# KCL-BMEIS/VS_Seg

Measured on AMD Instinct MI355X. Metric: train_patches_per_sec_fwd_bwd_384x128x128, higher is better.
Workload: dtype bf16; 1 GPU; BASELINE config 2: 2.5D attention-UNet fwd + Dice_spvPA(attention+hardness) + bwd + Adam on random 384x128x128 patches, batch 4 per GPU, dropout 0.1, random-init weights; global_batch=4, patch=384x128x128, parallelism=dp1

## Files before the change

vs_seg_amd/csrc/bn_bwd.h:

```cpp
#pragma once
#include "common.h"

struct BnBwdC8 {
  float sc[8], sh[8], mu[8], k1i[8], kc[8], kd[8];
};

__device__ __forceinline__ void bn_bwd_consts(BnBwdC8& c, const float* __restrict__ mean, const float* __restrict__ invstd, const float* __restrict__ gamma, const float* __restrict__ scale,
                                              const float* __restrict__ shift, const float* __restrict__ mean_dz, const float* __restrict__ mean_dzx, int ch0, float inv_keep) {
#pragma unroll
  for (int j = 0; j < 8; ++j) {
    const float is = invstd[ch0 + j], k1 = gamma[ch0 + j] * is;
    c.sc[j] = scale[ch0 + j];
    c.sh[j] = shift[ch0 + j];
    c.mu[j] = mean[ch0 + j];
    c.k1i[j] = k1 * inv_keep;
    c.kc[j] = -(k1 * mean_dzx[ch0 + j]) * is;
    c.kd[j] = -(k1 * mean_dz[ch0 + j]);
  }
}

__device__ __forceinline__ void bn_fwd_act8(const f8& y, unsigned keep, float alpha, float inv_keep, const float (&sc)[8], const float (&sh)[8], f8& o) {
#pragma unroll
  for (int j = 0; j < 8; ++j) {
    float z = y.v[j] * sc[j] + sh[j];
    z = ((keep >> j) & 1u) ? z * inv_keep : 0.f;
    o.v[j] = z > 0.f ? z : alpha * z;
  }
}

__device__ __forceinline__ void bn_bwd_dy8(const f8& y, const f8& g, unsigned keep, float alpha, const BnBwdC8& c, f8& o) {
#pragma unroll
  for (int j = 0; j < 8; ++j) {
    const float z = y.v[j] * c.sc[j] + c.sh[j];
    const float dd = z > 0.f ? g.v[j] : alpha * g.v[j];
    const float t = ((keep >> j) & 1u) ? dd : 0.f;
    o.v[j] = __builtin_fmaf(c.k1i[j], t, __builtin_fmaf(c.kc[j], y.v[j] - c.mu[j], c.kd[j]));
  }
}

__device__ __forceinline__ f8 bf16x8_to_f8(const uint4 u) {
  return f8{{__uint_as_float(u.x << 16), __uint_as_float(u.x & 0xffff0000u), __uint_as_float(u.y << 16), __uint_as_float(u.y & 0xffff0000u),
             __uint_as_float(u.z << 16), __uint_as_float(u.z & 0xffff0000u), __uint_as_float(u.w << 16), __uint_as_float(u.w & 0xffff0000u)}};
}
__device__ __forceinline__ uint4 f8_to_bf16x8(const f8& a) {
  uint4 u;
  u.x = f2bf2(a.v[0], a.v[1]);
  u.y = f2bf2(a.v[2], a.v[3]);
  u.z = f2bf2(a.v[4], a.v[5]);
  u.w = f2bf2(a.v[6], a.v[7]);
  return u;
}
```

vs_seg_amd/csrc/elementwise.hip:

```cpp
#define VSSEG_NT_STORES
#define VSSEG_NT_LOADS
#include "common.h"
#include "bn_bwd.h"
#include <algorithm>
#include <type_traits>

#define DISPATCH_T(dtype, ...)                         \
  do {                                                 \
    if ((dtype) == VSSEG_F32) { typedef float T; __VA_ARGS__; } \
    else { typedef bf16_t T; __VA_ARGS__; }            \
  } while (0)

static inline int split_of(const vsseg_tensor& t) { return t.ptr2 ? t.csplit : 0x7fffffff; }
static inline bool two_part_ok(const vsseg_tensor& t) {
  return !t.ptr2 || (t.csplit > 0 && t.csplit < t.c && t.csplit % 16 == 0 && t.pitch >= t.csplit && t.pitch >= t.c - t.csplit);
}
#define VSSEG_ONE_PART(name, ...)                                                                     \
  do {                                                                                                \
    const vsseg_tensor* ts_[] = {__VA_ARGS__};                                                        \
    for (const vsseg_tensor* t_ : ts_) VSSEG_CHECK(!t_->ptr2, name ": two-part tensors are not supported here"); \
  } while (0)

static inline int block_for_cgs(int cgs) {
  int a = cgs, b = 64;
// ... 221 lines not shown
#pragma unroll
      for (int j = 0; j < 8; ++j) r.v[j] = x1 * w1[j] + b1[j];
    }
    bn_fwd_act8(x, keep, alpha, inv_keep, sc, sh, x);
    if constexpr (RES != 0) {
#pragma unroll
      for (int j = 0; j < 8; ++j) x.v[j] += r.v[j];
    }
    st8(out + v * op + c, x);
  }
}
static inline int bn_fwd_grid(int64_t items, int cgs) {
  int g = grid_for(items, 256, 16384);
  g = (g + cgs - 1) / cgs * cgs;
  return g;
}
extern "C" int vsseg_bn_act_fwd(vsseg_tensor y, const float* scale, const float* shift, const float* alpha, float p_drop, uint64_t seed, uint32_t salt,
                                vsseg_tensor res, int32_t has_res, vsseg_tensor out, uint8_t* keep_out, void* stream) {
  VSSEG_ONE_PART("vsseg_bn_act_fwd", &y, &res, &out);
  VSSEG_CHECK(y.ptr && out.ptr && scale && shift && alpha && y.c % 8 == 0 && y.pitch % 8 == 0 && out.pitch % 8 == 0 && out.c == y.c && out.dtype == y.dtype, "vsseg_bn_act_fwd: bad arguments");
  VSSEG_CHECK(!has_res || (res.ptr && res.dtype == y.dtype && res.c == y.c && res.pitch % 8 == 0), "vsseg_bn_act_fwd: bad residual");
  VSSEG_CHECK(p_drop >= 0.f && p_drop < 1.f, "vsseg_bn_act_fwd: dropout p out of range");
  int64_t nv = tensor_voxels(y);
  int cgs = y.c / 8;
  dim3 g(bn_fwd_grid(nv * cgs, cgs)), b(256);
  DISPATCH_T(y.dtype, if (has_res) hipLaunchKernelGGL((bn_act_fwd_kernel<T, 1>), g, b, 0, as_stream(stream), (const T*)y.ptr, y.pitch, scale, shift, alpha, p_drop, seed, salt, (const T*)res.ptr, res.pitch, (T*)out.ptr, out.pitch, cgs, nv, (const float*)nullptr, (const float*)nullptr, keep_out);
             else hipLaunchKernelGGL((bn_act_fwd_kernel<T, 0>), g, b, 0, as_stream(stream), (const T*)y.ptr, y.pitch, scale, shift, alpha, p_drop, seed, salt, (const T*)nullptr, 0, (T*)out.ptr, out.pitch, cgs, nv, (const float*)nullptr, (const float*)nullptr, keep_out));
  VSSEG_LAUNCH_CHECK("vsseg_bn_act_fwd");
  return VSSEG_OK;
}
extern "C" int vsseg_bn_act_fwd_res1(vsseg_tensor y, const float* scale, const float* shift, const float* alpha, float p_drop, uint64_t seed, uint32_t salt,
                                     const void* x1, const float* res_w, const float* res_b, vsseg_tensor out, uint8_t* keep_out, void* stream) {
  VSSEG_ONE_PART("vsseg_bn_act_fwd_res1", &y, &out);
  VSSEG_CHECK(y.ptr && out.ptr && scale && shift && alpha && x1 && res_w && res_b && y.c % 8 == 0 && y.pitch % 8 == 0 && out.pitch % 8 == 0 && out.c == y.c && out.dtype == y.dtype, "vsseg_bn_act_fwd_res1: bad arguments");
  VSSEG_CHECK(p_drop >= 0.f && p_drop < 1.f, "vsseg_bn_act_fwd_res1: dropout p out of range");
  int64_t nv = tensor_voxels(y);
  int cgs = y.c / 8;
  dim3 g(bn_fwd_grid(nv * cgs, cgs)), b(256);
  DISPATCH_T(y.dtype, hipLaunchKernelGGL((bn_act_fwd_kernel<T, 2>), g, b, 0, as_stream(stream), (const T*)y.ptr, y.pitch, scale, shift, alpha, p_drop, seed, salt, (const T*)x1, 0, (T*)out.ptr, out.pitch, cgs, nv, res_w, res_b, keep_out));
  VSSEG_LAUNCH_CHECK("vsseg_bn_act_fwd_res1");
  return VSSEG_OK;
}

__global__ void dropout_mask_kernel(float* mask, int64_t n8, float p, uint64_t seed, uint32_t salt) {
  if (p > 0.f) dropout_resolve_seed(seed, salt);
  for (int64_t i = blockIdx.x * (int64_t)blockDim.x + threadIdx.x; i < n8; i += (int64_t)gridDim.x * blockDim.x) {
    unsigned keep = p > 0.f ? dropout_keep8(seed, salt, (uint64_t)i, p) : 0xffu;
    for (int j = 0; j < 8; ++j) mask[i * 8 + j] = (float)((keep >> j) & 1u);
  }
}
extern "C" int vsseg_dropout_mask(float* mask, int64_t nvox, int32_t c, float p_drop, uint64_t seed, uint32_t salt, void* stream) {
  VSSEG_CHECK(mask && c % 8 == 0, "vsseg_dropout_mask: bad arguments");
  int64_t n8 = nvox * (c / 8);
  hipLaunchKernelGGL(dropout_mask_kernel, dim3(grid_for(n8, 256)), dim3(256), 0, as_stream(stream), mask, n8, p_drop, seed, salt);
  VSSEG_LAUNCH_CHECK("vsseg_dropout_mask");
  return VSSEG_OK;
}

struct BnBwdArgs {
  const float *mean, *invstd, *gamma, *beta, *scale, *shift, *alpha;
  float p_drop;
  uint64_t seed;
  uint32_t salt;
};
__device__ __forceinline__ float bn_bwd_elem8(const f8& y, const f8& da, int c, int64_t i, const BnBwdArgs& a, float alpha, f8& dz, f8& xh) {
  const float inv_keep = 1.f / (1.f - a.p_drop);
  unsigned keep = a.p_drop > 0.f ? dropout_keep8(a.seed, a.salt, (uint64_t)i, a.p_drop) : 0xffu;
  float dal = 0.f;
#pragma unroll
  for (int j = 0; j < 8; ++j) {
    float xhat = (y.v[j] - a.mean[c + j]) * a.invstd[c + j];
    float z = y.v[j] * a.scale[c + j] + a.shift[c + j];
    bool k = (keep >> j) & 1u;
    float d = k ? z * inv_keep : 0.f;
    float g = da.v[j];
    float dd = d > 0.f ? g : alpha * g;
    if (d < 0.f) dal += g * d;
    dz.v[j] = k ? dd * inv_keep : 0.f;
    xh.v[j] = xhat;
  }
  return dal;
}

template <typename T> struct Raw8;
template <> struct Raw8<bf16_t> {
  uint4 u;
  static __device__ __forceinline__ Raw8 ld(const bf16_t* p) {
    Raw8 r;
#ifdef VSSEG_NT_LOADS
    typedef unsigned u32x4 __attribute__((ext_vector_type(4)));
    const u32x4 t = __builtin_nontemporal_load(reinterpret_cast<const u32x4*>(p));
    r.u = make_uint4(t[0], t[1], t[2], t[3]);
#else
    r.u = *reinterpret_cast<const uint4*>(p);
#endif
    return r;
  }
  __device__ __forceinline__ f8 cvt() const {
    return f8{{__uint_as_float(u.x << 16), __uint_as_float(u.x & 0xffff0000u), __uint_as_float(u.y << 16), __uint_as_float(u.y & 0xffff0000u),
               __uint_as_float(u.z << 16), __uint_as_float(u.z & 0xffff0000u), __uint_as_float(u.w << 16), __uint_as_float(u.w & 0xffff0000u)}};
  }
};
template <> struct Raw8<float> {
  f8 v;
  static __device__ __forceinline__ Raw8 ld(const float* p) { Raw8 r; r.v = ld8(p); return r; }
  __device__ __forceinline__ f8 cvt() const { return v; }
};

template <typename T, int U>
__global__ __launch_bounds__(1024) void bn_act_bwd_reduce_kernel(const T* __restrict__ y, int yp, const T* __restrict__ dout, int dp, BnBwdArgs a, int cgs, int64_t nvox, double* __restrict__ sums, int stride, double* __restrict__ alpha_acc,
                                                               const uint8_t* __restrict__ keep_in, unsigned* fxflag) {
  extern __shared__ float red[];
  const int C = cgs * 8, RW = 3 * C + 1, nw = (blockDim.x + 63) >> 6;
  for (int i = threadIdx.x; i < nw * RW; i += blockDim.x) red[i] = 0.f;
  __syncthreads();
  const float alpha = *a.alpha;
  if (a.p_drop > 0.f && keep_in == nullptr) dropout_resolve_seed(a.seed, a.salt);
  const int64_t gt = blockIdx.x * (int64_t)blockDim.x + threadIdx.x, nthreads = (int64_t)gridDim.x * blockDim.x;
  const int cg = (int)(gt % cgs);
  const int c = cg * 8;
  float sc[8], sh[8], mu[8];
#pragma unroll
  for (int j = 0; j < 8; ++j) { sc[j] = a.scale[c + j]; sh[j] = a.shift[c + j]; mu[j] = a.mean[c + j]; }
  const bool drop = a.p_drop > 0.f;
  const float inv_keep = 1.f / (1.f - a.p_drop);
  float s1[8] = {0, 0, 0, 0, 0, 0, 0, 0}, s2[8] = {0, 0, 0, 0, 0, 0, 0, 0}, s3[8] = {0, 0, 0, 0, 0, 0, 0, 0}, dal = 0.f;
  const int64_t vstep = nthreads / cgs;
  auto one = [&](const f8& yy, const f8& da, unsigned keep) {
#pragma unroll
    for (int j = 0; j < 8; ++j) {
      const float z = yy.v[j] * sc[j] + sh[j];
      const bool k = (keep >> j) & 1u;
      const float d = k ? z * inv_keep : 0.f;
      const float g = da.v[j];
      const float dd = d > 0.f ? g : alpha * g;
      if (d < 0.f) dal += g * d;
      const float dz = k ? dd * inv_keep : 0.f;
      s1[j] += dz; s2[j] += dz * (yy.v[j] - mu[j]); s3[j] += g;
    }
  };
  auto sweep = [&](auto src_c) {
    constexpr int SRC = decltype(src_c)::value;
    auto mask_of = [&](int64_t vv) -> unsigned {
      if constexpr (SRC == 0) return 0xffu;
      else if constexpr (SRC == 1) return (unsigned)keep_in[vv * cgs + cg];
      else return dropout_keep8(a.seed, a.salt, (uint64_t)(vv * cgs + cg), a.p_drop);
    };
    int64_t v = gt / cgs;
    for (; v + (U - 1) * vstep < nvox; v += U * vstep) {
      Raw8<T> yv[U], dv[U];
      unsigned kp[U];
#pragma unroll
      for (int u = 0; u < U; ++u) { yv[u] = Raw8<T>::ld(y + (v + u * vstep) * yp + c); dv[u] = Raw8<T>::ld(dout + (v + u * vstep) * dp + c); kp[u] = mask_of(v + u * vstep); }
#pragma unroll
      for (int u = 0; u < U; ++u) one(yv[u].cvt(), dv[u].cvt(), kp[u]);
    }
    for (; v < nvox; v += vstep) one(ld8(y + v * yp + c), ld8(dout + v * dp + c), mask_of(v));
  };
  if (!drop) sweep(std::integral_constant<int, 0>{});
  else if (keep_in != nullptr) sweep(std::integral_constant<int, 1>{});
  else sweep(std::integral_constant<int, 2>{});
  float* rw = red + (threadIdx.x >> 6) * RW;
#pragma unroll
  for (int j = 0; j < 8; ++j) { atomicAdd(&rw[c + j], s1[j]); atomicAdd(&rw[C + c + j], s2[j]); atomicAdd(&rw[2 * C + c + j], s3[j]); }
  dal = wave_sum(dal);
  if ((threadIdx.x & 63) == 0) rw[3 * C] = dal;
  __syncthreads();
  auto wsum = [&](int i) { float v = 0.f; for (int w = 0; w < nw; ++w) v += red[w * RW + i]; return v; };
  const int shard = blockIdx.x % VSSEG_STAT_SHARDS;
  for (int i = threadIdx.x; i < 3 * C; i += blockDim.x) {
    const int which = i / C, ch = i % C;
    double val = (double)wsum(i);
    if (which == 1) val *= (double)a.invstd[ch];
    vsseg_fx_add(&sums[(int64_t)shard * 3 * stride + which * stride + ch], val, VSSEG_FX_GRAD, fxflag);
  }
  if (threadIdx.x == 0) vsseg_fx_add(&alpha_acc[shard], (double)wsum(3 * C), VSSEG_FX_GRAD, fxflag);
}
extern "C" int vsseg_bn_act_bwd_reduce(vsseg_tensor y, vsseg_tensor dout, const float* mean, const float* invstd, const float* gamma, const float* beta, const float* scale, const float* shift, const float* alpha,
                                       float p_drop, uint64_t seed, uint32_t salt, double* sums, int32_t stride, double* alpha_acc, const uint8_t* keep_in, void* stream) {
  VSSEG_ONE_PART("vsseg_bn_act_bwd_reduce", &y, &dout);
  VSSEG_CHECK(y.ptr && dout.ptr && y.dtype == dout.dtype && y.c == dout.c && y.c % 8 == 0 && y.pitch % 8 == 0 && dout.pitch % 8 == 0 && sums && alpha_acc && stride >= y.c, "vsseg_bn_act_bwd_reduce: bad arguments");
  int cgs = y.c / 8, blk = block_for_cgs(cgs);
  VSSEG_CHECK(blk > 0, "vsseg_bn_act_bwd_reduce: unsupported channel count %d", y.c);
  int64_t nv = tensor_voxels(y);
  BnBwdArgs a{mean, invstd, gamma, beta, scale, shift, alpha, p_drop, seed, salt};
  size_t lds = (size_t)((blk + 63) / 64) * (3 * y.c + 1) * sizeof(float);
  const int64_t items = nv * cgs;
  const int budget = 65536;
  const int cap = (int)std::min<int64_t>(256 * 8, std::max<int64_t>(192, std::min<int64_t>(items / ((int64_t)blk * 16), y.c <= 16 ? 256 * 3 : budget / (3 * y.c))));
  int grid = grid_for((nv * cgs + 1) / 2, blk, cap);
  VSSEG_FX_FLAG(fxflag, "vsseg_bn_act_bwd_reduce");
  DISPATCH_T(y.dtype, hipLaunchKernelGGL((bn_act_bwd_reduce_kernel<T, 2>), dim3(grid), dim3(blk), lds, as_stream(stream), (const T*)y.ptr, y.pitch, (const T*)dout.ptr, dout.pitch, a, cgs, nv, sums, stride, alpha_acc, keep_in, fxflag));
  VSSEG_LAUNCH_CHECK("vsseg_bn_act_bwd_reduce");
  return VSSEG_OK;
}

__global__ void bn_act_bwd_finalize_kernel(const double* __restrict__ sums, int stride, const double* __restrict__ alpha_acc, int c, double count, float* dgamma, float* dbeta, float* dalpha, float* mean_dz, float* mean_dzx, float* dres_bias, const unsigned* fxflag) {
  __shared__ double part[4];
  const int ch = blockIdx.x, sh = threadIdx.x;
  const double* base = sums + (int64_t)sh * 3 * stride + ch;
  const double s = block256_sum_d(vsseg_fx_get(&base[0], VSSEG_FX_GRAD), part) + vsseg_fx_poison(fxflag);
  const double q = block256_sum_d(vsseg_fx_get(&base[stride], VSSEG_FX_GRAD), part) + vsseg_fx_poison(fxflag);
  const double r = block256_sum_d(vsseg_fx_get(&base[2 * stride], VSSEG_FX_GRAD), part) + vsseg_fx_poison(fxflag);
  double a = 0.0;
  if (ch == 0) a = block256_sum_d(vsseg_fx_get(&alpha_acc[sh], VSSEG_FX_GRAD), part);
  if (threadIdx.x != 0) return;
  if (ch == 0) *dalpha += (float)(a + vsseg_fx_poison(fxflag));
  if (dres_bias) dres_bias[ch] += (float)r;
  dbeta[ch] += (float)s;
  dgamma[ch] += (float)q;
  mean_dz[ch] = (float)(s / count);
  mean_dzx[ch] = (float)(q / count);
}
extern "C" int vsseg_bn_act_bwd_finalize(const double* sums, int32_t stride, const double* alpha_acc, int32_t c, double count, float* dgamma, float* dbeta, float* dalpha,
                                         float* mean_dz, float* mean_dzx, float* dres_bias, void* stream) {
  VSSEG_CHECK(sums && alpha_acc && dgamma && dbeta && dalpha && mean_dz && mean_dzx && c > 0, "vsseg_bn_act_bwd_finalize: bad arguments");
  VSSEG_FX_FLAG(fxflag, "vsseg_bn_act_bwd_finalize");
  hipLaunchKernelGGL(bn_act_bwd_finalize_kernel, dim3(c), dim3(256), 0, as_stream(stream), sums, stride, alpha_acc, c, count, dgamma, dbeta, dalpha, mean_dz, mean_dzx, dres_bias, fxflag);
  VSSEG_LAUNCH_CHECK("vsseg_bn_act_bwd_finalize");
  return VSSEG_OK;
}

template <typename T>
__global__ void bn_act_bwd_apply_kernel(const T* __restrict__ y, int yp, const T* __restrict__ dout, int dp, BnBwdArgs a, const float* __restrict__ mean_dz, const float* __restrict__ mean_dzx,
                                        T* __restrict__ dy, int dyp, int cgs, int64_t nvox, const uint8_t* __restrict__ keep_in) {
  const int64_t gt = blockIdx.x * (int64_t)blockDim.x + threadIdx.x, nthreads = (int64_t)gridDim.x * blockDim.x;
  const int cg = (int)(gt % cgs), c = cg * 8;
  const int64_t vstep = nthreads / cgs;
  const float alpha = *a.alpha, inv_keep = 1.f / (1.f - a.p_drop);
  BnBwdC8 k;
  bn_bwd_consts(k, a.mean, a.invstd, a.gamma, a.scale, a.shift, mean_dz, mean_dzx, c, inv_keep);
  const bool drop = a.p_drop > 0.f;
  if (drop && keep_in == nullptr) dropout_resolve_seed(a.seed, a.salt);
  auto one = [&](const f8& yy, const f8& da, unsigned keep, int64_t v) {
    f8 o;
    bn_bwd_dy8(yy, da, keep, alpha, k, o);
    st8(dy + v * dyp + c, o);
  };
  auto sweep = [&](auto src_c) {
    constexpr int SRC = decltype(src_c)::value;
    auto mask_of = [&](int64_t vv) -> unsigned {
      if constexpr (SRC == 0) return 0xffu;
      else if constexpr (SRC == 1) return (unsigned)keep_in[vv * cgs + cg];
      else return dropout_keep8(a.seed, a.salt, (uint64_t)(vv * cgs + cg), a.p_drop);
    };
    int64_t v = gt / cgs;
    for (; v + vstep < nvox; v += 2 * vstep) {
      const f8 y0 = ld8(y + v * yp + c), d0 = ld8(dout + v * dp + c);
      const f8 y1 = ld8(y + (v + vstep) * yp + c), d1 = ld8(dout + (v + vstep) * dp + c);
      const unsigned m0 = mask_of(v), m1 = mask_of(v + vstep);
      one(y0, d0, m0, v);
      one(y1, d1, m1, v + vstep);
    }
    if (v < nvox) one(ld8(y + v * yp + c), ld8(dout + v * dp + c), mask_of(v), v);
  };
  if (!drop) sweep(std::integral_constant<int, 0>{});
  else if (keep_in != nullptr) sweep(std::integral_constant<int, 1>{});
  else sweep(std::integral_constant<int, 2>{});
}

extern "C" int vsseg_bn_act_bwd_apply(vsseg_tensor y, vsseg_tensor dout, const float* mean, const float* invstd, const float* gamma, const float* beta, const float* scale, const float* shift, const float* alpha,
                                      float p_drop, uint64_t seed, uint32_t salt, const float* mean_dz, const float* mean_dzx, vsseg_tensor dy, const uint8_t* keep_in, void* stream) {
  VSSEG_ONE_PART("vsseg_bn_act_bwd_apply", &y, &dout, &dy);
  VSSEG_CHECK(y.ptr && dout.ptr && dy.ptr && y.dtype == dout.dtype && y.dtype == dy.dtype && y.c == dout.c && y.c == dy.c && y.c % 8 == 0 && y.pitch % 8 == 0 && dout.pitch % 8 == 0 && dy.pitch % 8 == 0,
              "vsseg_bn_act_bwd_apply: bad arguments");
  int cgs = y.c / 8, blk = block_for_cgs(cgs);
  VSSEG_CHECK(blk > 0, "vsseg_bn_act_bwd_apply: unsupported channel count %d", y.c);
  int64_t nv = tensor_voxels(y);
  BnBwdArgs a{mean, invstd, gamma, beta, scale, shift, alpha, p_drop, seed, salt};
  DISPATCH_T(y.dtype, hipLaunchKernelGGL(bn_act_bwd_apply_kernel<T>, dim3(grid_for((nv * cgs + 1) / 2, blk, 256 * 8)), dim3(blk), 0, as_stream(stream), (const T*)y.ptr, y.pitch, (const T*)dout.ptr, dout.pitch, a, mean_dz, mean_dzx, (T*)dy.ptr, dy.pitch, cgs, nv, keep_in));
  VSSEG_LAUNCH_CHECK("vsseg_bn_act_bwd_apply");
  return VSSEG_OK;
}

template <typename T>
__global__ void att_apply_fwd_kernel(const T* __restrict__ x, const T* __restrict__ x2, int xsplit, int xp, const float* __restrict__ att, T* __restrict__ out, int op, int cgs, int64_t nvox) {
  const int64_t total = nvox * cgs;
  for (int64_t i = blockIdx.x * (int64_t)blockDim.x + threadIdx.x; i < total; i += (int64_t)gridDim.x * blockDim.x) {
    int64_t v = i / cgs;
    int c = (int)(i - v * cgs) * 8;
    const float g = 1.f + att[v];
    f8 a = c >= xsplit ? ld8(x2 + v * xp + (c - xsplit)) : ld8(x + v * xp + c);
#pragma unroll
    for (int j = 0; j < 8; ++j) a.v[j] *= g;
    st8(out + v * op + c, a);
  }
}
extern "C" int vsseg_att_apply_fwd(vsseg_tensor x, const float* att, vsseg_tensor out, void* stream) {
  VSSEG_CHECK(x.ptr && att && out.ptr && x.dtype == out.dtype && x.c == out.c && x.c % 8 == 0 && x.pitch % 8 == 0 && out.pitch % 8 == 0 && !out.ptr2, "vsseg_att_apply_fwd: bad arguments");
  VSSEG_CHECK(two_part_ok(x), "vsseg_att_apply_fwd: bad two-part x");
  int cgs = x.c / 8;
  int64_t nv = tensor_voxels(x);
  DISPATCH_T(x.dtype, hipLaunchKernelGGL(att_apply_fwd_kernel<T>, dim3(grid_for(nv * cgs, 256)), dim3(256), 0, as_stream(stream), (const T*)x.ptr, (const T*)x.ptr2, split_of(x), x.pitch, att, (T*)out.ptr, out.pitch, cgs, nv));
  VSSEG_LAUNCH_CHECK("vsseg_att_apply_fwd");
  return VSSEG_OK;
}

template <typename T, bool ACC, int G>
__global__ void att_apply_bwd_kernel(const T* __restrict__ x0, const T* __restrict__ x1, int xsplit, int xp, const float* __restrict__ att, const T* __restrict__ dout, int dp, const float* __restrict__ datt_ext,
                                     T* __restrict__ dx0, T* __restrict__ dx1, int dxsplit, int dxp, T* __restrict__ dpre, int dprep, int cgs, int64_t nvox, float* __restrict__ dbias, T* __restrict__ dpre1, int skip_dx) {
  const int sub = threadIdx.x % G;
  const T* x = sub * 8 >= xsplit ? x1 - xsplit : x0;
  T* dx = sub * 8 >= dxsplit ? dx1 - dxsplit : dx0;
  const int64_t vstep = (int64_t)gridDim.x * (blockDim.x / G);
  float bsum = 0.f;
  for (int64_t v0 = blockIdx.x * (int64_t)(blockDim.x / G); v0 < nvox; v0 += vstep) {
    const int64_t v = v0 + threadIdx.x / G;
    const bool live = v < nvox;
    float dot = 0.f, a = 0.f;
    if (live) {
      a = att[v];
      if (sub < cgs) {
        const float g = 1.f + a;
        f8 xx = ld8(x + v * xp + sub * 8), d = ld8(dout + v * dp + sub * 8), o;
        if (ACC) o = ld8(dx + v * dxp + sub * 8);
#pragma unroll
        for (int j = 0; j < 8; ++j) {
          dot += d.v[j] * xx.v[j];
          o.v[j] = ACC ? o.v[j] + d.v[j] * g : d.v[j] * g;
        }
        if (!skip_dx) st8(dx + v * dxp + sub * 8, o);
      }
    }
#pragma unroll
    for (int o = G / 2; o > 0; o >>= 1) dot += __shfl_xor(dot, o, 64);
    if (live && sub == 0) {
      if (datt_ext) dot += datt_ext[v];
      const float r = dot * a * (1.f - a);
      if (dpre) st8(dpre + v * dprep, f8{{r, 0, 0, 0, 0, 0, 0, 0}});
      if (dpre1) Elem<T>::st(dpre1 + v, r);
      bsum += r;
    }
  }
  if (dbias) {
    bsum = wave_sum(bsum);
    __shared__ float part[16];
    if ((threadIdx.x & 63) == 0) part[threadIdx.x >> 6] = bsum;
    __syncthreads();
    if (threadIdx.x == 0) {
      float t = 0.f;
      for (int w = 0; w < (int)(blockDim.x >> 6); ++w) t += part[w];
      atomicAdd(dbias, t);
    }
  }
}
template <typename T, bool ACC> static void att_bwd_launch(int G, dim3 g, dim3 b, hipStream_t s, vsseg_tensor x, const float* att, const T* dout, int dp, const float* de, vsseg_tensor dx, T* dpre, int dprep, int cgs, int64_t nv, float* dbias, T* dpre1, int skip_dx) {
#define VSSEG_ATT_BWD(GG) hipLaunchKernelGGL((att_apply_bwd_kernel<T, ACC, GG>), g, b, 0, s, (const T*)x.ptr, (const T*)x.ptr2, split_of(x), x.pitch, att, dout, dp, de, (T*)dx.ptr, (T*)dx.ptr2, split_of(dx), dx.pitch, dpre, dprep, cgs, nv, dbias, dpre1, skip_dx)
  switch (G) {
    case 1: VSSEG_ATT_BWD(1); break;
    case 2: VSSEG_ATT_BWD(2); break;
    case 4: VSSEG_ATT_BWD(4); break;
    case 8: VSSEG_ATT_BWD(8); break;
    case 16: VSSEG_ATT_BWD(16); break;
// ... 83 lines not shown
```

vs_seg_amd/csrc/wgrad_narrow.hip:

```cpp
#define VSSEG_NT_LOADS
#include "common.h"
#include "bn_bwd.h"

struct WnK {
  const void* t;
  const void* s;
  float* dw;
  float* slab;
  int bias;
  int tpitch, C, cgs;
  int n, X, Y, Z, yq;
  int sign;
  int64_t stride_c;
  int64_t items;
  const void* da;
  const unsigned char* keep;
  const float *mean, *invstd, *gamma, *scale, *shift, *alpha, *mean_dz, *mean_dzx;
  float inv_keep;
  int dapitch;
};

template <typename T> __device__ __forceinline__ float wn_ld(const T* p);
template <> __device__ __forceinline__ float wn_ld<float>(const float* p) { return *p; }
template <> __device__ __forceinline__ float wn_ld<bf16_t>(const bf16_t* p) { return bf2f(*p); }

template <typename T, int K3, bool BN = false>
__global__ __launch_bounds__(256) void wgrad_narrow_kernel(const WnK k) {
  constexpr int NT = K3 * K3, ROWS = K3 == 3 ? 6 : 4, R = K3 / 2;
  __shared__ float red[4][NT * 64 + 1];
  const int tid = threadIdx.x, C = k.C, cgs = k.cgs;
  float bsum = 0.f;
  const int64_t gt = blockIdx.x * 256ll + tid, nthreads = (int64_t)gridDim.x * 256;
  const int cg = (int)(gt % cgs);
  const int64_t step = nthreads / cgs;
  const T* tp = reinterpret_cast<const T*>(k.t) + cg * 8;
  const T* sp = reinterpret_cast<const T*>(k.s);
  const T* dap = BN ? reinterpret_cast<const T*>(k.da) + cg * 8 : nullptr;
  BnBwdC8 bc;
  float alpha = 0.f;
  if constexpr (BN) {
    bn_bwd_consts(bc, k.mean, k.invstd, k.gamma, k.scale, k.shift, k.mean_dz, k.mean_dzx, cg * 8, k.inv_keep);
    alpha = *k.alpha;
  }
  const int X = k.X, Y = k.Y, Z = k.Z;
  float acc[NT][8];
#pragma unroll
  for (int t = 0; t < NT; ++t)
#pragma unroll
    for (int c = 0; c < 8; ++c) acc[t][c] = 0.f;
  const unsigned first = (unsigned)(gt / cgs), ustep = (unsigned)step, uitems = (unsigned)k.items;
  const int YQ = k.yq, ZY = Z * Y;
  int z = (int)(first % (unsigned)Z), yq = (int)((first / (unsigned)Z) % (unsigned)YQ), x = (int)((first / (unsigned)(Z * YQ)) % (unsigned)X), n = (int)(first / (unsigned)(Z * YQ * X));
  const int sz = (int)(ustep % (unsigned)Z), syq = (int)((ustep / (unsigned)Z) % (unsigned)YQ), sx = (int)((ustep / (unsigned)(Z * YQ)) % (unsigned)X), sn = (int)(ustep / (unsigned)(Z * YQ * X));
  const int my_items = first < uitems ? (int)((uitems - 1u - first) / ustep) + 1 : 0;
  const int64_t trow = (int64_t)Z * k.tpitch;
  for (int it = 0; it < my_items; ++it) {
    const int y0 = yq * 4;
    const int v0 = ((n * X + x) * Y + y0) * Z + z;
    const T* t0 = tp + (int64_t)v0 * k.tpitch;
    f8 tv[4];
#pragma unroll
    for (int i = 0; i < 4; ++i) tv[i] = ld8(t0 + i * trow);
    if constexpr (BN) {
      const T* d0 = dap + (int64_t)v0 * k.dapitch;
      const int64_t darow = (int64_t)Z * k.dapitch;
      f8 dv[4];
      unsigned kp[4];
#pragma unroll
      for (int i = 0; i < 4; ++i) {
        dv[i] = ld8(d0 + i * darow);
        kp[i] = k.keep ? (unsigned)k.keep[(int64_t)(v0 + i * Z) * cgs + cg] : 0xffu;
      }
#pragma unroll
      for (int i = 0; i < 4; ++i) {
        f8 o;
        bn_bwd_dy8(tv[i], dv[i], kp[i], alpha, bc, o);
        if constexpr (sizeof(T) == 2) tv[i] = bf16x8_to_f8(f8_to_bf16x8(o));
        else tv[i] = o;
      }
    }
#pragma unroll
    for (int dxi = 0; dxi < K3; ++dxi) {
      const int xs = x + dxi - R;
      const bool xok = (unsigned)xs < (unsigned)X;
      const T* s0 = sp + (v0 + (xok ? (dxi - R) * ZY : 0));
      float sr[ROWS];
#pragma unroll
      for (int j = 0; j < ROWS; ++j) {
        const int ys = y0 - R + j;
        const bool yok = (unsigned)ys < (unsigned)Y;
        const float v = wn_ld<T>(s0 + (yok ? (j - R) * Z : 0));
        sr[j] = (xok && yok) ? v : 0.f;
      }
      if (dxi == R) bsum += (sr[R] + sr[R + 1]) + (sr[R + 2] + sr[R + 3]);
#pragma unroll
      for (int i = 0; i < 4; ++i)
#pragma unroll
        for (int dyi = 0; dyi < K3; ++dyi)
#pragma unroll
          for (int c = 0; c < 8; ++c) acc[dxi * K3 + dyi][c] += tv[i].v[c] * sr[i + dyi];
    }
    z += sz; if (z >= Z) { z -= Z; ++yq; }
    yq += syq; if (yq >= YQ) { yq -= YQ; ++x; }
    x += sx; if (x >= X) { x -= X; ++n; }
    n += sn;
  }
  const int wave = tid >> 6;
#pragma unroll
  for (int t = 0; t < NT; ++t)
#pragma unroll
    for (int c = 0; c < 8; ++c) {
      float v = acc[t][c];
      for (int o = 32; o >= cgs; o >>= 1) v += __shfl_xor(v, o, 64);
      if ((tid & 63) < cgs) red[wave][t * C + cg * 8 + c] = v;
    }
  bsum = wave_sum(cg == 0 ? bsum : 0.f);
  if ((tid & 63) == 0) red[wave][NT * C] = bsum;
  __syncthreads();
  const int row = NT * C + (k.bias ? 1 : 0);
  float* slab = k.slab + (int64_t)blockIdx.x * row;
  for (int i = tid; i < row; i += 256) slab[i] = (red[0][i] + red[1][i]) + (red[2][i] + red[3][i]);
}

__global__ __launch_bounds__(VSSEG_SLAB_THREADS) void wgrad_narrow_reduce_kernel(const float* __restrict__ slab, int nblk, int C, int K3, int sign, float* __restrict__ dw, int64_t stride_c, float* __restrict__ dbias) {
  __shared__ float lds[VSSEG_SLAB_THREADS];
  const int NT = K3 * K3, R = K3 / 2;
  const int64_t total = (int64_t)NT * C + (dbias ? 1 : 0);
  const int64_t i = (int64_t)blockIdx.x * 64 + (threadIdx.x & 63);
  const float s = vsseg_slab_sum(slab, total, i, nblk, lds);
  if (threadIdx.x >= 64 || i >= total) return;
  if (i == (int64_t)NT * C) { *dbias += s; return; }
  const int t = (int)i / C, c = (int)i - t * C;
  const int dx = t / K3 - R, dy = t % K3 - R;
  const int widx = (sign * dx + R) * K3 + (sign * dy + R);
  dw[(int64_t)c * stride_c + widx] += s;
}

static int wgrad_narrow_impl(vsseg_tensor t, const void* s, int32_t k3, int32_t sign, float* dw, int64_t stride_c, float* dbias, float* scratch, int64_t scratch_elems, void* stream, const WnK* bn);
extern "C" int vsseg_wgrad_narrow(vsseg_tensor t, const void* s, int32_t k3, int32_t sign, float* dw, int64_t stride_c, float* dbias, float* scratch, int64_t scratch_elems, void* stream) {
  return wgrad_narrow_impl(t, s, k3, sign, dw, stride_c, dbias, scratch, scratch_elems, stream, nullptr);
}
extern "C" int vsseg_wgrad_narrow_bn(vsseg_tensor y, vsseg_tensor dout, const uint8_t* keep, const float* mean, const float* invstd, const float* gamma, const float* scale, const float* shift, const float* alpha,
                                     const float* mean_dz, const float* mean_dzx, float p_drop, const void* s, float* dw, int64_t stride_c, float* scratch, int64_t scratch_elems, void* stream) {
  VSSEG_CHECK(y.ptr && dout.ptr && !dout.ptr2 && mean && invstd && gamma && scale && shift && alpha && mean_dz && mean_dzx, "vsseg_wgrad_narrow_bn: null pointer");
  VSSEG_CHECK(y.dtype == VSSEG_BF16 && dout.dtype == VSSEG_BF16 && dout.c == y.c && dout.pitch % 8 == 0 && dout.n == y.n && dout.x == y.x && dout.y == y.y && dout.z == y.z, "vsseg_wgrad_narrow_bn: y / dout must be bf16 tensors of one shape");
  VSSEG_CHECK(p_drop >= 0.f && p_drop < 1.f && (p_drop == 0.f || keep), "vsseg_wgrad_narrow_bn: dropout needs the keep-mask bytes of the forward");
  WnK bn;
  bn.da = dout.ptr; bn.dapitch = dout.pitch; bn.keep = p_drop > 0.f ? keep : nullptr;
  bn.mean = mean; bn.invstd = invstd; bn.gamma = gamma; bn.scale = scale; bn.shift = shift; bn.alpha = alpha; bn.mean_dz = mean_dz; bn.mean_dzx = mean_dzx;
  bn.inv_keep = 1.f / (1.f - p_drop);
  return wgrad_narrow_impl(y, s, 3, 1, dw, stride_c, nullptr, scratch, scratch_elems, stream, &bn);
}
static int wgrad_narrow_impl(vsseg_tensor t, const void* s, int32_t k3, int32_t sign, float* dw, int64_t stride_c, float* dbias, float* scratch, int64_t scratch_elems, void* stream, const WnK* bn) {
  VSSEG_CHECK(!dbias || sign == -1, "vsseg_wgrad_narrow: the bias gradient (sum of the one-channel dY) belongs to the C -> 1 case (sign = -1)");
  VSSEG_CHECK(t.ptr && s && dw && scratch && !t.ptr2, "vsseg_wgrad_narrow: bad pointers (two-part tensors are not supported)");
  VSSEG_CHECK(k3 == 1 || k3 == 3, "vsseg_wgrad_narrow: 3x3x1 or 1x1x1 kernels only (k3 = %d)", k3);
  VSSEG_CHECK(sign == 1 || sign == -1, "vsseg_wgrad_narrow: sign must be +1 or -1");
  VSSEG_CHECK(t.c % 8 == 0 && t.c >= 8 && t.c <= 64 && 64 % (t.c / 8) == 0 && t.pitch % 8 == 0, "vsseg_wgrad_narrow: channel count %d must be 8, 16, 32 or 64", t.c);
  VSSEG_CHECK(t.y % 4 == 0, "vsseg_wgrad_narrow: y extent %d must be a multiple of 4", t.y);
  WnK k;
  k.t = t.ptr; k.s = s; k.dw = dw;
  k.tpitch = t.pitch; k.C = t.c; k.cgs = t.c / 8;
  k.n = t.n; k.X = t.x; k.Y = t.y; k.Z = t.z; k.yq = t.y / 4;
  k.sign = sign; k.stride_c = stride_c;
  k.items = (int64_t)t.n * t.x * k.yq * t.z;
  VSSEG_CHECK((int64_t)t.n * t.x * t.y * t.z < (1ll << 31), "vsseg_wgrad_narrow: more than 2^31 voxels");
  int grid = grid_for(k.items * k.cgs / 16, 256, 256 * 3);
  k.bias = dbias ? 1 : 0;
  const int64_t cap = scratch_elems / (k3 * k3 * t.c + 1);
  VSSEG_CHECK(cap >= 1, "vsseg_wgrad_narrow: scratch too small");
  if (grid > cap) grid = (int)cap;
  k.slab = scratch;
  k.da = nullptr; k.keep = nullptr;
  if (bn) {
    k.da = bn->da; k.dapitch = bn->dapitch; k.keep = bn->keep; k.inv_keep = bn->inv_keep;
    k.mean = bn->mean; k.invstd = bn->invstd; k.gamma = bn->gamma; k.scale = bn->scale; k.shift = bn->shift; k.alpha = bn->alpha; k.mean_dz = bn->mean_dz; k.mean_dzx = bn->mean_dzx;
    hipLaunchKernelGGL((wgrad_narrow_kernel<bf16_t, 3, true>), dim3(grid), dim3(256), 0, as_stream(stream), k);
  } else if (t.dtype == VSSEG_F32) {
    if (k3 == 3) hipLaunchKernelGGL((wgrad_narrow_kernel<float, 3>), dim3(grid), dim3(256), 0, as_stream(stream), k);
    else hipLaunchKernelGGL((wgrad_narrow_kernel<float, 1>), dim3(grid), dim3(256), 0, as_stream(stream), k);
  } else {
    if (k3 == 3) hipLaunchKernelGGL((wgrad_narrow_kernel<bf16_t, 3>), dim3(grid), dim3(256), 0, as_stream(stream), k);
    else hipLaunchKernelGGL((wgrad_narrow_kernel<bf16_t, 1>), dim3(grid), dim3(256), 0, as_stream(stream), k);
  }
  VSSEG_LAUNCH_CHECK("vsseg_wgrad_narrow");
  const int total = k3 * k3 * t.c + (dbias ? 1 : 0);
  hipLaunchKernelGGL(wgrad_narrow_reduce_kernel, dim3((total + 63) / 64), dim3(VSSEG_SLAB_THREADS), 0, as_stream(stream), (const float*)scratch, grid, (int)t.c, (int)k3, (int)sign, dw, stride_c, dbias);
  VSSEG_LAUNCH_CHECK("vsseg_wgrad_narrow(reduce)");
  return VSSEG_OK;
}
```

Baseline: 158.4 patches/s.

## Prefetch next item in BN-fused narrow wgrad and specialize BN-bwd apply kernel

The BN-fused path of the narrow weight-gradient kernel becomes software-pipelined: the raw bf16 loads of t, dout and the keep mask for the next item are issued before the current item is computed, so load latency overlaps the accumulation. The BN-backward apply kernel is templated on the dropout-mask source and block size, which removes runtime branching and lets launch bounds match the block. The wgrad grid cap now comes from a queried occupancy times the CU count instead of a fixed value. Holding prefetched data raises register pressure, which may lower occupancy.

```diff
diff --git a/vs_seg_amd/csrc/bn_bwd.h b/vs_seg_amd/csrc/bn_bwd.h
--- a/vs_seg_amd/csrc/bn_bwd.h
+++ b/vs_seg_amd/csrc/bn_bwd.h
@@ -42,6 +42,27 @@
   return f8{{__uint_as_float(u.x << 16), __uint_as_float(u.x & 0xffff0000u), __uint_as_float(u.y << 16), __uint_as_float(u.y & 0xffff0000u),
              __uint_as_float(u.z << 16), __uint_as_float(u.z & 0xffff0000u), __uint_as_float(u.w << 16), __uint_as_float(u.w & 0xffff0000u)}};
 }
+template <typename T> struct Raw8;
+template <> struct Raw8<bf16_t> {
+  uint4 u;
+  static __device__ __forceinline__ Raw8 ld(const bf16_t* p) {
+    Raw8 r;
+#ifdef VSSEG_NT_LOADS
+    typedef unsigned u32x4 __attribute__((ext_vector_type(4)));
+    const u32x4 t = __builtin_nontemporal_load(reinterpret_cast<const u32x4*>(p));
+    r.u = make_uint4(t[0], t[1], t[2], t[3]);
+#else
+    r.u = *reinterpret_cast<const uint4*>(p);
+#endif
+    return r;
+  }
+  __device__ __forceinline__ f8 cvt() const { return bf16x8_to_f8(u); }
+};
+template <> struct Raw8<float> {
+  f8 v;
+  static __device__ __forceinline__ Raw8 ld(const float* p) { Raw8 r; r.v = ld8(p); return r; }
+  __device__ __forceinline__ f8 cvt() const { return v; }
+};
 __device__ __forceinline__ uint4 f8_to_bf16x8(const f8& a) {
   uint4 u;
   u.x = f2bf2(a.v[0], a.v[1]);
diff --git a/vs_seg_amd/csrc/elementwise.hip b/vs_seg_amd/csrc/elementwise.hip
--- a/vs_seg_amd/csrc/elementwise.hip
+++ b/vs_seg_amd/csrc/elementwise.hip
@@ -327,31 +327,6 @@
   return dal;
 }
 
-template <typename T> struct Raw8;
-template <> struct Raw8<bf16_t> {
-  uint4 u;
-  static __device__ __forceinline__ Raw8 ld(const bf16_t* p) {
-    Raw8 r;
-#ifdef VSSEG_NT_LOADS
-    typedef unsigned u32x4 __attribute__((ext_vector_type(4)));
-    const u32x4 t = __builtin_nontemporal_load(reinterpret_cast<const u32x4*>(p));
-    r.u = make_uint4(t[0], t[1], t[2], t[3]);
-#else
-    r.u = *reinterpret_cast<const uint4*>(p);
-#endif
-    return r;
-  }
-  __device__ __forceinline__ f8 cvt() const {
-    return f8{{__uint_as_float(u.x << 16), __uint_as_float(u.x & 0xffff0000u), __uint_as_float(u.y << 16), __uint_as_float(u.y & 0xffff0000u),
-               __uint_as_float(u.z << 16), __uint_as_float(u.z & 0xffff0000u), __uint_as_float(u.w << 16), __uint_as_float(u.w & 0xffff0000u)}};
-  }
-};
-template <> struct Raw8<float> {
-  f8 v;
-  static __device__ __forceinline__ Raw8 ld(const float* p) { Raw8 r; r.v = ld8(p); return r; }
-  __device__ __forceinline__ f8 cvt() const { return v; }
-};
-
 template <typename T, int U>
 __global__ __launch_bounds__(1024) void bn_act_bwd_reduce_kernel(const T* __restrict__ y, int yp, const T* __restrict__ dout, int dp, BnBwdArgs a, int cgs, int64_t nvox, double* __restrict__ sums, int stride, double* __restrict__ alpha_acc,
                                                                const uint8_t* __restrict__ keep_in, unsigned* fxflag) {
@@ -466,42 +441,50 @@
   return VSSEG_OK;
 }
 
-template <typename T>
-__global__ void bn_act_bwd_apply_kernel(const T* __restrict__ y, int yp, const T* __restrict__ dout, int dp, BnBwdArgs a, const float* __restrict__ mean_dz, const float* __restrict__ mean_dzx,
-                                        T* __restrict__ dy, int dyp, int cgs, int64_t nvox, const uint8_t* __restrict__ keep_in) {
+#define DISPATCH_BLK_(SRC, blk, L)          \
+  do {                                      \
+    if ((blk) <= 256) { L(SRC, 256); }      \
+    else if ((blk) <= 384) { L(SRC, 384); } \
+    else { L(SRC, 1024); }                  \
+  } while (0)
+#define DISPATCH_SRC_BLK(src, blk, L)              \
+  do {                                             \
+    if ((src) == 0) DISPATCH_BLK_(0, blk, L);      \
+    else if ((src) == 1) DISPATCH_BLK_(1, blk, L); \
+    else DISPATCH_BLK_(2, blk, L);                 \
+  } while (0)
+template <typename T, int SRC, int BLK>
+__global__ __launch_bounds__(BLK) void bn_act_bwd_apply_kernel(const T* __restrict__ y, int yp, const T* __restrict__ dout, int dp, BnBwdArgs a, const float* __restrict__ mean_dz, const float* __restrict__ mean_dzx,
+                                                             T* __restrict__ dy, int dyp, int cgs, int64_t nvox, const uint8_t* __restrict__ keep_in) {
   const int64_t gt = blockIdx.x * (int64_t)blockDim.x + threadIdx.x, nthreads = (int64_t)gridDim.x * blockDim.x;
   const int cg = (int)(gt % cgs), c = cg * 8;
   const int64_t vstep = nthreads / cgs;
   const float alpha = *a.alpha, inv_keep = 1.f / (1.f - a.p_drop);
   BnBwdC8 k;
   bn_bwd_consts(k, a.mean, a.invstd, a.gamma, a.scale, a.shift, mean_dz, mean_dzx, c, inv_keep);
-  const bool drop = a.p_drop > 0.f;
-  if (drop && keep_in == nullptr) dropout_resolve_seed(a.seed, a.salt);
+  if constexpr (SRC == 2) dropout_resolve_seed(a.seed, a.salt);
   auto one = [&](const f8& yy, const f8& da, unsigned keep, int64_t v) {
     f8 o;
     bn_bwd_dy8(yy, da, keep, alpha, k, o);
     st8(dy + v * dyp + c, o);
   };
-  auto sweep = [&](auto src_c) {
-    constexpr int SRC = decltype(src_c)::value;
-    auto mask_of = [&](int64_t vv) -> unsigned {
-      if constexpr (SRC == 0) return 0xffu;
-      else if constexpr (SRC == 1) return (unsigned)keep_in[vv * cgs + cg];
-      else return dropout_keep8(a.seed, a.salt, (uint64_t)(vv * cgs + cg), a.p_drop);
-    };
-    int64_t v = gt / cgs;
-    for (; v + vstep < nvox; v += 2 * vstep) {
-      const f8 y0 = ld8(y + v * yp + c), d0 = ld8(dout + v * dp + c);
-      const f8 y1 = ld8(y + (v + vstep) * yp + c), d1 = ld8(dout + (v + vstep) * dp + c);
-      const unsigned m0 = mask_of(v), m1 = mask_of(v + vstep);
-      one(y0, d0, m0, v);
-      one(y1, d1, m1, v + vstep);
-    }
-    if (v < nvox) one(ld8(y + v * yp + c), ld8(dout + v * dp + c), mask_of(v), v);
+  auto mask_ld = [&](int64_t vv) -> unsigned {
+    if constexpr (SRC == 1) return (unsigned)keep_in[vv * cgs + cg];
+    else return 0xffu;
   };
-  if (!drop) sweep(std::integral_constant<int, 0>{});
-  else if (keep_in != nullptr) sweep(std::integral_constant<int, 1>{});
-  else sweep(std::integral_constant<int, 2>{});
+  auto mask_of = [&](int64_t vv, unsigned loaded) -> unsigned {
+    if constexpr (SRC == 2) return dropout_keep8(a.seed, a.salt, (uint64_t)(vv * cgs + cg), a.p_drop);
+    else return loaded;
+  };
+  int64_t v = gt / cgs;
+  for (; v + vstep < nvox; v += 2 * vstep) {
+    const f8 y0 = ld8(y + v * yp + c), d0 = ld8(dout + v * dp + c);
+    const f8 y1 = ld8(y + (v + vstep) * yp + c), d1 = ld8(dout + (v + vstep) * dp + c);
+    const unsigned m0 = mask_ld(v), m1 = mask_ld(v + vstep);
+    one(y0, d0, mask_of(v, m0), v);
+    one(y1, d1, mask_of(v + vstep, m1), v + vstep);
+  }
+  if (v < nvox) one(ld8(y + v * yp + c), ld8(dout + v * dp + c), mask_of(v, mask_ld(v)), v);
 }
 
 extern "C" int vsseg_bn_act_bwd_apply(vsseg_tensor y, vsseg_tensor dout, const float* mean, const float* invstd, const float* gamma, const float* beta, const float* scale, const float* shift, const float* alpha,
@@ -513,7 +496,10 @@
   VSSEG_CHECK(blk > 0, "vsseg_bn_act_bwd_apply: unsupported channel count %d", y.c);
   int64_t nv = tensor_voxels(y);
   BnBwdArgs a{mean, invstd, gamma, beta, scale, shift, alpha, p_drop, seed, salt};
-  DISPATCH_T(y.dtype, hipLaunchKernelGGL(bn_act_bwd_apply_kernel<T>, dim3(grid_for((nv * cgs + 1) / 2, blk, 256 * 8)), dim3(blk), 0, as_stream(stream), (const T*)y.ptr, y.pitch, (const T*)dout.ptr, dout.pitch, a, mean_dz, mean_dzx, (T*)dy.ptr, dy.pitch, cgs, nv, keep_in));
+  const int src = p_drop > 0.f ? (keep_in ? 1 : 2) : 0, grid = grid_for((nv * cgs + 1) / 2, blk, 256 * 8);
+#define LAUNCH_(SRC, BLK) hipLaunchKernelGGL((bn_act_bwd_apply_kernel<T, SRC, BLK>), dim3(grid), dim3(blk), 0, as_stream(stream), (const T*)y.ptr, y.pitch, (const T*)dout.ptr, dout.pitch, a, mean_dz, mean_dzx, (T*)dy.ptr, dy.pitch, cgs, nv, keep_in)
+  DISPATCH_T(y.dtype, DISPATCH_SRC_BLK(src, blk, LAUNCH_));
+#undef LAUNCH_
   VSSEG_LAUNCH_CHECK("vsseg_bn_act_bwd_apply");
   return VSSEG_OK;
 }
diff --git a/vs_seg_amd/csrc/wgrad_narrow.hip b/vs_seg_amd/csrc/wgrad_narrow.hip
--- a/vs_seg_amd/csrc/wgrad_narrow.hip
+++ b/vs_seg_amd/csrc/wgrad_narrow.hip
@@ -54,56 +54,101 @@
   const int sz = (int)(ustep % (unsigned)Z), syq = (int)((ustep / (unsigned)Z) % (unsigned)YQ), sx = (int)((ustep / (unsigned)(Z * YQ)) % (unsigned)X), sn = (int)(ustep / (unsigned)(Z * YQ * X));
   const int my_items = first < uitems ? (int)((uitems - 1u - first) / ustep) + 1 : 0;
   const int64_t trow = (int64_t)Z * k.tpitch;
-  for (int it = 0; it < my_items; ++it) {
-    const int y0 = yq * 4;
-    const int v0 = ((n * X + x) * Y + y0) * Z + z;
-    const T* t0 = tp + (int64_t)v0 * k.tpitch;
-    f8 tv[4];
-#pragma unroll
-    for (int i = 0; i < 4; ++i) tv[i] = ld8(t0 + i * trow);
-    if constexpr (BN) {
+  if constexpr (BN) {
+    const int64_t darow = (int64_t)Z * k.dapitch;
+    struct WnItem {
+      Raw8<T> t[4], d[4];
+      unsigned kp[4] = {0xffu, 0xffu, 0xffu, 0xffu};
+    };
+    const bool has_keep = k.keep != nullptr;
+    auto issue = [&](WnItem& b, int v0) {
+      const T* t0 = tp + (int64_t)v0 * k.tpitch;
+#pragma unroll
+      for (int i = 0; i < 4; ++i) b.t[i] = Raw8<T>::ld(t0 + i * trow);
       const T* d0 = dap + (int64_t)v0 * k.dapitch;
-      const int64_t darow = (int64_t)Z * k.dapitch;
-      f8 dv[4];
-      unsigned kp[4];
+#pragma unroll
+      for (int i = 0; i < 4; ++i) b.d[i] = Raw8<T>::ld(d0 + i * darow);
+      if (has_keep) {
+#pragma unroll
+        for (int i = 0; i < 4; ++i) b.kp[i] = (unsigned)k.keep[(int64_t)(v0 + i * Z) * cgs + cg];
+      }
+    };
+    WnItem nxt;
+    if (my_items > 0) issue(nxt, ((n * X + x) * Y + yq * 4) * Z + z);
+    for (int it = 0; it < my_items; ++it) {
+      const WnItem cur = nxt;
+      const bool last = it + 1 >= my_items;
+      const int y0 = yq * 4;
+      const int v0 = ((n * X + x) * Y + y0) * Z + z;
+      const int xc = x;
+      z += sz; if (z >= Z) { z -= Z; ++yq; }
+      yq += syq; if (yq >= YQ) { yq -= YQ; ++x; }
+      x += sx; if (x >= X) { x -= X; ++n; }
+      n += sn;
+      float sr[K3][ROWS];
+#pragma unroll
+      for (int dxi = 0; dxi < K3; ++dxi) {
+        const bool xok = (unsigned)(xc + dxi - R) < (unsigned)X;
+        const T* s0 = sp + (v0 + (xok ? (dxi - R) * ZY : 0));
+#pragma unroll
+        for (int j = 0; j < ROWS; ++j) {
+          const bool yok = (unsigned)(y0 - R + j) < (unsigned)Y;
+          int off = yok ? (j - R) * Z : 0;
+          asm volatile("" : "+v"(off));
+          const float v = wn_ld<T>(s0 + off);
+          sr[dxi][j] = (xok && yok) ? v : 0.f;
+        }
+      }
+      asm volatile("" ::: "memory");
+      issue(nxt, last ? v0 : ((n * X + x) * Y + yq * 4) * Z + z);
+      bsum += (sr[R][R] + sr[R][R + 1]) + (sr[R][R + 2] + sr[R][R + 3]);
 #pragma unroll
       for (int i = 0; i < 4; ++i) {
-        dv[i] = ld8(d0 + i * darow);
-        kp[i] = k.keep ? (unsigned)k.keep[(int64_t)(v0 + i * Z) * cgs + cg] : 0xffu;
-      }
-#pragma unroll
-      for (int i = 0; i < 4; ++i) {
-        f8 o;
-        bn_bwd_dy8(tv[i], dv[i], kp[i], alpha, bc, o);
-        if constexpr (sizeof(T) == 2) tv[i] = bf16x8_to_f8(f8_to_bf16x8(o));
-        else tv[i] = o;
+        f8 tv;
+        bn_bwd_dy8(cur.t[i].cvt(), cur.d[i].cvt(), cur.kp[i], alpha, bc, tv);
+        if constexpr (sizeof(T) == 2) tv = bf16x8_to_f8(f8_to_bf16x8(tv));
+#pragma unroll
+        for (int dxi = 0; dxi < K3; ++dxi)
+#pragma unroll
+          for (int dyi = 0; dyi < K3; ++dyi)
+#pragma unroll
+            for (int c = 0; c < 8; ++c) acc[dxi * K3 + dyi][c] += tv.v[c] * sr[dxi][i + dyi];
       }
     }
-#pragma unroll
-    for (int dxi = 0; dxi < K3; ++dxi) {
-      const int xs = x + dxi - R;
-      const bool xok = (unsigned)xs < (unsigned)X;
-      const T* s0 = sp + (v0 + (xok ? (dxi - R) * ZY : 0));
-      float sr[ROWS];
-#pragma unroll
-      for (int j = 0; j < ROWS; ++j) {
-        const int ys = y0 - R + j;
-        const bool yok = (unsigned)ys < (unsigned)Y;
-        const float v = wn_ld<T>(s0 + (yok ? (j - R) * Z : 0));
-        sr[j] = (xok && yok) ? v : 0.f;
-      }
-      if (dxi == R) bsum += (sr[R] + sr[R + 1]) + (sr[R + 2] + sr[R + 3]);
-#pragma unroll
-      for (int i = 0; i < 4; ++i)
-#pragma unroll
-        for (int dyi = 0; dyi < K3; ++dyi)
-#pragma unroll
-          for (int c = 0; c < 8; ++c) acc[dxi * K3 + dyi][c] += tv[i].v[c] * sr[i + dyi];
+  } else {
+    for (int it = 0; it < my_items; ++it) {
+      const int y0 = yq * 4;
+      const int v0 = ((n * X + x) * Y + y0) * Z + z;
+      const T* t0 = tp + (int64_t)v0 * k.tpitch;
+      f8 tv[4];
+#pragma unroll
+      for (int i = 0; i < 4; ++i) tv[i] = ld8(t0 + i * trow);
+#pragma unroll
+      for (int dxi = 0; dxi < K3; ++dxi) {
+        const int xs = x + dxi - R;
+        const bool xok = (unsigned)xs < (unsigned)X;
+        const T* s0 = sp + (v0 + (xok ? (dxi - R) * ZY : 0));
+        float sr[ROWS];
+#pragma unroll
+        for (int j = 0; j < ROWS; ++j) {
+          const int ys = y0 - R + j;
+          const bool yok = (unsigned)ys < (unsigned)Y;
+          const float v = wn_ld<T>(s0 + (yok ? (j - R) * Z : 0));
+          sr[j] = (xok && yok) ? v : 0.f;
+        }
+        if (dxi == R) bsum += (sr[R] + sr[R + 1]) + (sr[R + 2] + sr[R + 3]);
+#pragma unroll
+        for (int i = 0; i < 4; ++i)
+#pragma unroll
+          for (int dyi = 0; dyi < K3; ++dyi)
+#pragma unroll
+            for (int c = 0; c < 8; ++c) acc[dxi * K3 + dyi][c] += tv[i].v[c] * sr[i + dyi];
+      }
+      z += sz; if (z >= Z) { z -= Z; ++yq; }
+      yq += syq; if (yq >= YQ) { yq -= YQ; ++x; }
+      x += sx; if (x >= X) { x -= X; ++n; }
+      n += sn;
     }
-    z += sz; if (z >= Z) { z -= Z; ++yq; }
-    yq += syq; if (yq >= YQ) { yq -= YQ; ++x; }
-    x += sx; if (x >= X) { x -= X; ++n; }
-    n += sn;
   }
   const int wave = tid >> 6;
 #pragma unroll
@@ -150,6 +195,16 @@
   bn.mean = mean; bn.invstd = invstd; bn.gamma = gamma; bn.scale = scale; bn.shift = shift; bn.alpha = alpha; bn.mean_dz = mean_dz; bn.mean_dzx = mean_dzx;
   bn.inv_keep = 1.f / (1.f - p_drop);
   return wgrad_narrow_impl(y, s, 3, 1, dw, stride_c, nullptr, scratch, scratch_elems, stream, &bn);
+}
+static int wn_resident_blocks() {
+  static int blocks = 0;
+  if (blocks == 0) {
+    int per_cu = 0, dev = 0, cus = 0;
+    if (hipOccupancyMaxActiveBlocksPerMultiprocessor(&per_cu, wgrad_narrow_kernel<bf16_t, 3, true>, 256, 0) != hipSuccess || per_cu < 1) { (void)hipGetLastError(); per_cu = 2; }
+    if (hipGetDevice(&dev) != hipSuccess || hipDeviceGetAttribute(&cus, hipDeviceAttributeMultiprocessorCount, dev) != hipSuccess || cus < 1) { (void)hipGetLastError(); cus = 256; }
+    blocks = per_cu * cus;
+  }
+  return blocks;
 }
 static int wgrad_narrow_impl(vsseg_tensor t, const void* s, int32_t k3, int32_t sign, float* dw, int64_t stride_c, float* dbias, float* scratch, int64_t scratch_elems, void* stream, const WnK* bn) {
   VSSEG_CHECK(!dbias || sign == -1, "vsseg_wgrad_narrow: the bias gradient (sum of the one-channel dY) belongs to the C -> 1 case (sign = -1)");
@@ -165,7 +220,7 @@
   k.sign = sign; k.stride_c = stride_c;
   k.items = (int64_t)t.n * t.x * k.yq * t.z;
   VSSEG_CHECK((int64_t)t.n * t.x * t.y * t.z < (1ll << 31), "vsseg_wgrad_narrow: more than 2^31 voxels");
-  int grid = grid_for(k.items * k.cgs / 16, 256, 256 * 3);
+  int grid = grid_for(k.items * k.cgs / 16, 256, wn_resident_blocks());
   k.bias = dbias ? 1 : 0;
   const int64_t cap = scratch_elems / (k3 * k3 * t.c + 1);
   VSSEG_CHECK(cap >= 1, "vsseg_wgrad_narrow: scratch too small");
```

Measured after the change: 158.5 patches/s (median of 2 runs). No clear change (+0.1%).
